# microsoft/YOLaT-VectorGraphicsRecognition

Measured on AMD Instinct MI355X. Metric: graphs_per_sec, higher is better.
Workload: dtype f32

## Files before the change

include/yolat_hip.h:

```cpp
#ifndef YOLAT_HIP_H
#define YOLAT_HIP_H

#include <stddef.h>
#include <stdint.h>

#ifdef __cplusplus
extern "C" {
#endif

typedef void* yolat_stream_t;

#define YOLAT_E_INVALID   (-1)
#define YOLAT_E_UNSUPPORTED (-2)

#define YOLAT_STATUS_EDGE_RANGE  1
#define YOLAT_STATUS_SEG_UNSORTED 2
#define YOLAT_STATUS_SEG_RANGE   4
#define YOLAT_STATUS_NOT_LOCAL   8


int yolat_abi_version(void);
const char* yolat_strerror(int code);


size_t yolat_csr_work_elems(int64_t N, int64_t E);
int yolat_coo_to_csr(const int64_t* edge, int64_t stride_e, int64_t stride_c, int64_t E, int64_t N,
                     int32_t* row_ptr, int32_t* perm, int32_t* src_csr, int32_t* dst_csr,
                     int32_t* work, int32_t* status, yolat_stream_t stream);

size_t yolat_csc_work_elems(int64_t N);
int yolat_csc_by_source(const int32_t* src_csr, int64_t E, int64_t N, int32_t* col_ptr,
                        int32_t* slots, int32_t* work, yolat_stream_t stream);

int yolat_expand_ranges(const int32_t* start, const int32_t* prefix, int64_t S, int64_t total, int32_t* out,
                        yolat_stream_t stream);
size_t yolat_subgraph_work_elems(int64_t N, int64_t n_sub);
int yolat_subgraph_reindex(const int32_t* node_ids, int64_t n_sub, int64_t N, const int64_t* edge,
                           int64_t stride_e, int64_t stride_c, const int32_t* edge_ids, int64_t m_sub,
                           const int64_t* bbox_idx, int64_t* edge_out, int64_t* bbox_idx_out, int32_t* work,
                           int32_t* status, yolat_stream_t stream);
int yolat_gather_rows_bytes(const void* src, int64_t src_row_bytes, const int32_t* idx, int64_t rows,
                            int64_t row_bytes, void* dst, int64_t dst_row_bytes, yolat_stream_t stream);

int yolat_fixup_offsets(int64_t* edge, int64_t E, const int64_t* edge_ptr, int64_t* bbox_idx, int64_t N,
                        const int64_t* node_ptr, const int64_t* node_off, const int64_t* prop_off, int64_t B,
                        yolat_stream_t stream);

int yolat_segment_ptr(const int64_t* bbox_idx, int64_t N, int64_t P, int32_t* seg_ptr,
                      int32_t* node_seg, int32_t* status, yolat_stream_t stream);

size_t yolat_graph_work_elems(int64_t N, int64_t E);
int yolat_graph_prepare(const int64_t* edge, int64_t stride_e, int64_t stride_c, const float* e_attr,
                        const int64_t* bbox_idx, int64_t E, int64_t N, int64_t P, int32_t* row_ptr,
                        int32_t* perm, int32_t* src_csr, int32_t* dst_csr, float* attr_csr,
                        int32_t* seg_ptr, int32_t* node_seg, int32_t* work, int32_t* status,
                        yolat_stream_t stream);

int yolat_graph_prepare_plan(int64_t N, int64_t E, int64_t other_wgs, int32_t* rows, int32_t* csr_wgs);

int yolat_gather_rows(const float* src, int64_t ld_src, const int32_t* idx, int64_t rows,
                      int64_t width, float* dst, int64_t ld_dst, yolat_stream_t stream);


#define YOLAT_STATS_ROWS 32
size_t yolat_bn_stats_elems(int64_t M, int64_t C);
int yolat_linear_fwd(const float* A, int64_t lda, int64_t M, int64_t K,
                     const float* a_scale, const float* a_shift, int a_relu,
                     const float* W, int64_t ldw, const float* bias, int64_t Nout,
                     const float* o_scale, const float* o_shift, int o_relu,
                     float* Y, int64_t ldy, int accumulate, float* stats, yolat_stream_t stream);

int yolat_linear_segmax_fwd(const float* A, int64_t lda, int64_t M, int64_t K, const float* W,
                            int64_t ldw, const float* bias, int64_t Nout, const float* o_scale,
                            const float* o_shift, const int32_t* node_seg, float* pool, int64_t ldpool,
                            yolat_stream_t stream);

int yolat_linear_fwd_wt(const float* A, int64_t lda, int64_t M, int64_t K,
                        const float* Wt, int64_t ldw, int64_t Nout,
                        float* Y, int64_t ldy, int accumulate, yolat_stream_t stream);

size_t yolat_linear_bwd_w_work_elems(int64_t M, int64_t Nout, int64_t K);
int yolat_linear_bwd_w(const float* dY, int64_t lddy, int64_t M, int64_t Nout,
                       const float* A, int64_t lda, int64_t K,
                       const float* a_scale, const float* a_shift, int a_relu,
                       float* dW, int64_t lddw, float* db, int accumulate,
                       float* partial, yolat_stream_t stream);

int yolat_bn_finalize(const float* stats, int64_t M, int64_t C, const float* gamma,
                      const float* beta, float* running_mean, float* running_var,
                      float momentum, float eps, float* save_mean, float* save_invstd,
                      float* scale, float* shift, yolat_stream_t stream);

int yolat_bn_eval_coeffs(const float* gamma, const float* beta, const float* running_mean,
                         const float* running_var, float eps, int64_t C, float* scale,
                         float* shift, yolat_stream_t stream);

int yolat_scale_shift_relu(const float* Y, int64_t ldy, int64_t M, int64_t C, const float* scale,
                           const float* shift, int relu, float* Z, int64_t ldz,
                           yolat_stream_t stream);

size_t yolat_bn_bwd_work_elems(int64_t M, int64_t C);
int yolat_bn_relu_bwd(const float* dZ, int64_t lddz, const float* Y, int64_t ldy, int64_t M,
                      int64_t C, const float* gamma, const float* save_mean,
                      const float* save_invstd, const float* scale, const float* shift, int relu,
                      float* dgamma, float* dbeta, int accumulate, float* dY, int64_t lddy,
                      float* work, yolat_stream_t stream);


int yolat_edge_lin1_fwd(const float* x, int64_t ldx, int64_t N, int64_t Cin,
                        const int32_t* src_csr, const int32_t* dst_csr, const float* attr_csr,
                        int64_t E, const float* W1, int64_t ldw, const float* b1, int64_t C,
                        const float* o_scale, const float* o_shift, int o_relu,
                        float* H1, int64_t ldh, float* stats, yolat_stream_t stream);

int yolat_edge_lin1_bwd_w(const float* dH1, int64_t lddh, int64_t E, int64_t C,
                          const float* x, int64_t ldx, int64_t N, int64_t Cin,
                          const int32_t* src_csr, const int32_t* dst_csr, const float* attr_csr,
                          float* dW1, int64_t lddw, float* db1, int accumulate, float* partial,
                          yolat_stream_t stream);

int yolat_edge_lin1_bwd_x(const float* dH1, int64_t lddh, int64_t E, int64_t C, const float* W1,
                          int64_t ldw, int64_t Cin, float* dG, int64_t lddg,
                          yolat_stream_t stream);

int yolat_edge_scatter_bwd(const float* dG, int64_t lddg, int64_t Cin, const int32_t* row_ptr,
                           const int32_t* col_ptr, const int32_t* slots, int64_t N, float* dX,
                           int64_t lddx, int accumulate, yolat_stream_t stream);

int yolat_edge_mlp2_eval(const float* x, int64_t ldx, int64_t N, int64_t Cin, const int32_t* src_csr,
                         const int32_t* dst_csr, const float* attr_csr, int64_t E, const float* W1,
                         const float* b1, const float* s1, const float* t1, const float* W2,
                         const float* b2, const float* s2, const float* t2, int64_t C, float* H2,
                         int64_t ldh, yolat_stream_t stream);

int yolat_graph_prepare_node_uv(const int64_t* edge, int64_t stride_e, int64_t stride_c, const float* e_attr,
                                const int64_t* bbox_idx, int64_t E, int64_t N, int64_t P, int32_t* row_ptr,
                                int32_t* perm, int32_t* src_csr, int32_t* dst_csr, float* attr_csr,
                                int32_t* seg_ptr, int32_t* node_seg, int32_t* work, int32_t* status, const float* x,
                                int64_t ldx, int64_t Cin, const float* Wuv, const float* uv_bias, const float* Wr,
                                const float* br,
                                const float* Wn, const float* bn, const float* sn, const float* tn, int64_t C,
                                float* UV, int64_t ld_uv, float* f_out, int64_t ld_fo, float* s_out, int64_t ld_so,
                                yolat_stream_t stream);

int yolat_conv_split_w1(const float* W1, int64_t Cin, int64_t C, float* Wuv, float* Wc4, yolat_stream_t stream);
int yolat_node_uv_eval(const float* f_in, int64_t ld_f, const float* s_in, int64_t ld_s, int64_t N, int64_t Cin,
                       const float* Wuv, const float* uv_bias, const float* Wr, const float* br, const float* Wn,
                       const float* bn, const float* sn, const float* tn, int64_t C, float* UV, int64_t ld_uv,
                       float* f_out, int64_t ld_fo, float* s_out, int64_t ld_so, yolat_stream_t stream);
int yolat_edge_uv_lin1_fwd(const float* UV, int64_t ld_uv, const int32_t* src_csr, const int32_t* dst_csr,
                           const float* attr_csr, int64_t E, const float* Wc4, const float* b1, int64_t C,
                           float* H1, int64_t ldh, float* stats, yolat_stream_t stream);

// ... 486 lines not shown
```

yolat_vectorgraphicsrecognition_amd/_lib.py:

```python
import ctypes
import os

_HERE = os.path.dirname(os.path.abspath(__file__))
LIB_PATH = os.environ.get("YOLAT_LIB_PATH") or os.path.join(_HERE, "libyolat_hip.so")

c_p = ctypes.c_void_p
c_i64 = ctypes.c_int64
c_int = ctypes.c_int
c_f = ctypes.c_float
c_sz = ctypes.c_size_t

YOLAT_MAX_LAYERS = 8


class ConvEval(ctypes.Structure):
    _fields_ = ([("Cin", c_i64)] + [(n, c_p) for n in
                                    ("W1", "b1", "s1", "t1", "W2", "b2", "s2", "t2", "Wr", "br", "Wn", "bn", "sn", "tn",
                                     "Wuv", "Wc4", "Wuvf", "uvb", "Wc4f", "t2f")] +
                [("Wfr_x6", c_p * 3), ("tfr", c_p), ("Wn_x6", c_p * 3), ("tn_fold", c_p), ("Wnx", c_p), ("tnx", c_p)])


class ModelEval(ctypes.Structure):
    _fields_ = ([("n_blocks", ctypes.c_int32), ("n_blocks_out", ctypes.c_int32), ("n_classes", ctypes.c_int32),
                 ("reserved", ctypes.c_int32), ("C", c_i64), ("F", c_i64), ("H1", c_i64), ("H2", c_i64),
# ... 60 lines not shown
                ("node", TrainLin), ("bn_node", TrainBn)]


class TrainModel(ctypes.Structure):
    _fields_ = [("n_blocks", ctypes.c_int32), ("n_blocks_out", ctypes.c_int32), ("n_classes", ctypes.c_int32),
                ("half", ctypes.c_int32), ("C", c_i64), ("F", c_i64), ("H1", c_i64), ("H2", c_i64),
                ("conv", TrainConv * YOLAT_MAX_LAYERS), ("fus", TrainLin), ("fus_bn", TrainBn), ("fus_s", TrainLin),
                ("fus_s_bn", TrainBn), ("c1", TrainLin), ("c1_bn", TrainBn), ("c2", TrainLin), ("c2_bn", TrainBn),
                ("c3", TrainLin), ("param_base", c_p), ("grad_base", c_p)]


class AdamArgs(ctypes.Structure):
    _fields_ = [("exp_avg", c_p), ("exp_avg_sq", c_p), ("n", c_i64), ("step", c_i64), ("lr", c_f), ("beta1", c_f),
                ("beta2", c_f), ("eps", c_f), ("weight_decay", c_f), ("grad_scale", c_f)]


class PredictTree(ctypes.Structure):
    _fields_ = [("R", c_i64), ("Ctot", c_i64), ("B", c_i64), ("root_row", c_p), ("root_range", c_p), ("child_ptr", c_p),
                ("child_row", c_p), ("child_range", c_p), ("image_root_ptr", c_p)]


class GraphCsr(ctypes.Structure):
    _fields_ = [("row_ptr", c_p), ("src", c_p), ("dst", c_p), ("attr", c_p), ("seg_ptr", c_p), ("node_seg", c_p)]


SIGNATURES = {
    "yolat_abi_version": (c_int, []),
    "yolat_strerror": (ctypes.c_char_p, [c_int]),
    "yolat_csr_work_elems": (c_sz, [c_i64, c_i64]),
    "yolat_coo_to_csr": (c_int, [c_p, c_i64, c_i64, c_i64, c_i64, c_p, c_p, c_p, c_p, c_p, c_p, c_p]),
    "yolat_edge_mlp2_eval": (c_int, [c_p, c_i64, c_i64, c_i64, c_p, c_p, c_p, c_i64, c_p, c_p, c_p, c_p, c_p, c_p, c_p,
                                      c_p, c_i64, c_p, c_i64, c_p]),
    "yolat_node_side_eval": (c_int, [c_p, c_i64, c_p, c_i64, c_i64, c_i64, c_p, c_p, c_p, c_p, c_p, c_p, c_p, c_i64,
                                      c_p, c_i64, c_i64, c_p, c_i64, c_p, c_i64, c_p]),
    "yolat_fusion_pool_train_saved_elems": (c_sz, [c_i64, c_i64, c_i64]),
    "yolat_fusion_pool_train_work_elems": (c_sz, [c_i64, c_i64, c_i64, c_i64]),
    "yolat_fusion_pool_train_fwd": (c_int, [c_p, c_i64, c_i64, c_i64, c_p, c_p, c_i64, c_p, c_p, c_p, c_p, c_f, c_f,
                                             c_p, c_i64, c_p, c_i64, c_p, c_p, c_p, c_p]),
    "yolat_fusion_pool_train_bwd": (c_int, [c_p, c_i64, c_i64, c_i64, c_p, c_p, c_i64, c_p, c_p, c_p, c_p, c_i64, c_p,
                                             c_i64, c_p, c_p, c_p, c_p, c_p, c_i64, c_p, c_p]),
    "yolat_fusion_pool_train_bwd_parts": (c_int, [c_p, c_i64, c_i64, c_i64, c_p, c_p, c_i64, c_p, c_p, c_p, c_p, c_i64, c_p,
                                                   c_i64, c_p, c_p, c_p, c_p, c_p, c_i64, c_p, c_int, c_p]),
    "yolat_fusion_pool_train_fwd_bf16": (c_int, [c_p, c_i64, c_i64, c_i64, c_p, c_p, c_i64, c_p, c_p, c_p, c_p, c_f, c_f,
                                                  c_p, c_i64, c_p, c_i64, c_p, c_p, c_p, c_p]),
    "yolat_fusion_pool_train_bwd_parts_bf16": (c_int, [c_p, c_i64, c_i64, c_i64, c_p, c_p, c_i64, c_p, c_p, c_p, c_p, c_i64,
                                                        c_p, c_i64, c_p, c_p, c_p, c_p, c_p, c_i64, c_p, c_int, c_p]),
    "yolat_bt_linear_fwd": (c_int, [c_p, c_i64, c_i64, c_i64, c_p, c_p, c_int, c_p, c_i64, c_p, c_i64, c_p, c_i64, c_p, c_p]),
    "yolat_bt_linear_fwd_wt": (c_int, [c_p, c_i64, c_i64, c_i64, c_p, c_i64, c_i64, c_p, c_i64, c_int, c_p]),
    "yolat_bt_linear_bwd_w_work_elems": (c_sz, [c_i64, c_i64, c_i64]),
    "yolat_bt_linear_bwd_w": (c_int, [c_p, c_i64, c_i64, c_i64, c_p, c_i64, c_i64, c_p, c_p, c_int, c_p, c_i64, c_p, c_p,
                                       c_p]),
    "yolat_expand_ranges": (c_int, [c_p, c_p, c_i64, c_i64, c_p, c_p]),
    "yolat_subgraph_work_elems": (c_sz, [c_i64, c_i64]),
    "yolat_subgraph_reindex": (c_int, [c_p, c_i64, c_i64, c_p, c_i64, c_i64, c_p, c_i64, c_p, c_p, c_p, c_p, c_p, c_p]),
    "yolat_gather_rows_bytes": (c_int, [c_p, c_i64, c_p, c_i64, c_i64, c_p, c_i64, c_p]),
    "yolat_fixup_offsets": (c_int, [c_p, c_i64, c_p, c_p, c_i64, c_p, c_p, c_p, c_i64, c_p]),
    "yolat_conv_split_w1": (c_int, [c_p, c_i64, c_i64, c_p, c_p, c_p]),
    "yolat_node_uv_eval": (c_int, [c_p, c_i64, c_p, c_i64, c_i64, c_i64, c_p, c_p, c_p, c_p, c_p, c_p, c_p, c_p, c_i64,
                                    c_p, c_i64, c_p, c_i64, c_p, c_i64, c_p]),
    "yolat_edge_uv_mlp2_eval": (c_int, [c_p, c_i64, c_p, c_p, c_p, c_i64, c_p, c_p, c_p, c_p, c_p, c_p, c_p, c_p, c_i64,
                                         c_p, c_i64, c_p]),
    "yolat_edge_uv_mlp2_mean_eval": (c_int, [c_p, c_i64, c_p, c_p, c_p, c_p, c_i64, c_i64, c_p, c_p, c_p, c_p, c_p, c_p,
                                              c_p, c_p, c_i64, c_p, c_i64, c_p]),
    "yolat_edge_uv_mlp2_mean_eval_variant": (c_int, [c_p, c_i64, c_p, c_p, c_p, c_p, c_i64, c_i64, c_p, c_p, c_p, c_p,
                                                      c_p, c_p, c_p, c_p, c_i64, c_p, c_i64, c_int, c_p]),
    "yolat_edge_uv_sums": (c_int, [c_p, c_i64, c_p, c_p, c_p, c_i64, c_i64, c_p, c_i64, c_p]),
    "yolat_conv_merge_dw1": (c_int, [c_p, c_p, c_i64, c_i64, c_p, c_i64, c_int, c_p]),
    "yolat_fusion_pair_eval": (c_int, [c_p, c_i64, c_i64, c_i64, c_p, c_p, c_p, c_p, c_i64, c_p, c_p, c_i64, c_p, c_i64,
                                        c_i64, c_p, c_p, c_p, c_p, c_p, c_i64, c_p]),
    "yolat_graph_prepare_node_uv": (c_int, [c_p, c_i64, c_i64, c_p, c_p, c_i64, c_i64, c_i64] + [c_p] * 9 +
                                    [c_p, c_i64, c_i64] + [c_p] * 8 + [c_i64, c_p, c_i64, c_p, c_i64, c_p, c_i64, c_p]),
    "yolat_csc_work_elems": (c_sz, [c_i64]),
    "yolat_csc_by_source": (c_int, [c_p, c_i64, c_i64, c_p, c_p, c_p, c_p]),
    "yolat_segment_ptr": (c_int, [c_p, c_i64, c_i64, c_p, c_p, c_p, c_p]),
    "yolat_graph_work_elems": (c_sz, [c_i64, c_i64]),
    "yolat_graph_prepare": (c_int, [c_p, c_i64, c_i64, c_p, c_p, c_i64, c_i64, c_i64, c_p, c_p, c_p, c_p, c_p,
                                    c_p, c_p, c_p, c_p, c_p]),
    "yolat_graph_prepare_plan": (c_int, [c_i64, c_i64, c_i64, c_p, c_p]),
    "yolat_gather_rows": (c_int, [c_p, c_i64, c_p, c_i64, c_i64, c_p, c_i64, c_p]),
    "yolat_bn_stats_elems": (c_sz, [c_i64, c_i64]),
    "yolat_linear_fwd": (c_int, [c_p, c_i64, c_i64, c_i64, c_p, c_p, c_int,
                                 c_p, c_i64, c_p, c_i64, c_p, c_p, c_int,
                                 c_p, c_i64, c_int, c_p, c_p]),
    "yolat_linear_segmax_fwd": (c_int, [c_p, c_i64, c_i64, c_i64, c_p, c_i64, c_p, c_i64, c_p, c_p, c_p, c_p, c_i64,
                                        c_p]),
    "yolat_linear_fwd_wt": (c_int, [c_p, c_i64, c_i64, c_i64, c_p, c_i64, c_i64, c_p, c_i64, c_int, c_p]),
    "yolat_linear_bwd_w_work_elems": (c_sz, [c_i64, c_i64, c_i64]),
    "yolat_linear_bwd_w": (c_int, [c_p, c_i64, c_i64, c_i64, c_p, c_i64, c_i64, c_p, c_p, c_int,
                                   c_p, c_i64, c_p, c_int, c_p, c_p]),
    "yolat_bn_finalize": (c_int, [c_p, c_i64, c_i64, c_p, c_p, c_p, c_p, c_f, c_f, c_p, c_p, c_p, c_p, c_p]),
    "yolat_bn_eval_coeffs": (c_int, [c_p, c_p, c_p, c_p, c_f, c_i64, c_p, c_p, c_p]),
    "yolat_scale_shift_relu": (c_int, [c_p, c_i64, c_i64, c_i64, c_p, c_p, c_int, c_p, c_i64, c_p]),
    "yolat_bn_bwd_work_elems": (c_sz, [c_i64, c_i64]),
    "yolat_bn_relu_bwd": (c_int, [c_p, c_i64, c_p, c_i64, c_i64, c_i64, c_p, c_p, c_p, c_p, c_p, c_int,
                                  c_p, c_p, c_int, c_p, c_i64, c_p, c_p]),
    "yolat_edge_lin1_fwd": (c_int, [c_p, c_i64, c_i64, c_i64, c_p, c_p, c_p, c_i64, c_p, c_i64, c_p,
                                    c_i64, c_p, c_p, c_int, c_p, c_i64, c_p, c_p]),
    "yolat_edge_lin1_bwd_w": (c_int, [c_p, c_i64, c_i64, c_i64, c_p, c_i64, c_i64, c_i64, c_p, c_p, c_p,
                                      c_p, c_i64, c_p, c_int, c_p, c_p]),
    "yolat_edge_lin1_bwd_x": (c_int, [c_p, c_i64, c_i64, c_i64, c_p, c_i64, c_i64, c_p, c_i64, c_p]),
    "yolat_edge_scatter_bwd": (c_int, [c_p, c_i64, c_i64, c_p, c_p, c_p, c_i64, c_p, c_i64, c_int, c_p]),
    "yolat_csr_mean_fwd": (c_int, [c_p, c_i64, c_i64, c_p, c_p, c_int, c_p, c_i64, c_p, c_i64, c_int, c_p]),
    "yolat_csr_mean_bwd": (c_int, [c_p, c_i64, c_i64, c_p, c_p, c_i64, c_p, c_i64, c_p]),
    "yolat_segment_mean_fwd": (c_int, [c_p, c_i64, c_i64, c_p, c_p, c_int, c_p, c_i64, c_p, c_i64, c_p]),
    "yolat_segment_max_fwd": (c_int, [c_p, c_i64, c_i64, c_p, c_p, c_int, c_p, c_i64, c_i64, c_p, c_i64,
                                      c_p, c_p]),
    "yolat_pool_prepare": (c_int, [c_p, c_p, c_i64, c_i64, c_i64, c_p, c_i64, c_p, c_i64, c_p]),
    "yolat_segment_mean_bwd": (c_int, [c_p, c_i64, c_i64, c_p, c_p, c_i64, c_p, c_i64, c_p]),
    "yolat_segment_max_bwd": (c_int, [c_p, c_i64, c_i64, c_p, c_p, c_i64, c_p, c_i64, c_p]),
    "yolat_softmax_ce_work_elems": (c_sz, [c_i64]),
    "yolat_softmax_ce": (c_int, [c_p, c_i64, c_p, c_i64, c_i64, c_p, c_p, c_i64, c_p, c_p]),
    "yolat_sigmoid": (c_int, [c_p, c_i64, c_i64, c_i64, c_p, c_i64, c_p]),
    "yolat_sigmoid_bwd": (c_int, [c_p, c_i64, c_p, c_i64, c_i64, c_i64, c_p, c_i64, c_p]),
    "yolat_bce_work_elems": (c_sz, [c_i64]),
    "yolat_bce": (c_int, [c_p, c_i64, c_p, c_i64, c_i64, c_p, c_p, c_i64, c_p, c_p]),
    "yolat_sigmoid_bce": (c_int, [c_p, c_i64, c_p, c_i64, c_i64, c_p, c_p, c_i64, c_p, c_i64, c_p, c_p]),
    "yolat_adam_step": (c_int, [c_p, c_p, c_p, c_p, c_i64, c_f, c_f, c_f, c_f, c_f, c_i64, c_f, c_p]),
    "yolat_profile_enabled": (c_int, []),
    "yolat_profile_enable": (c_int, [c_int]),
    "yolat_profile_reset": (c_int, []),
    "yolat_profile_count": (c_int, []),
    "yolat_profile_get": (c_int, [c_int, ctypes.c_char_p, c_int, ctypes.POINTER(c_f), ctypes.POINTER(c_int),
                                  ctypes.POINTER(ctypes.c_double), ctypes.POINTER(ctypes.c_double)]),
    "yolat_forward_eval_workspace_bytes": (c_sz, [ctypes.POINTER(ModelEval), c_i64, c_i64, c_i64]),
    "yolat_forward_eval": (c_int, [ctypes.POINTER(ModelEval), c_p, c_i64, c_p, c_i64, c_i64, c_p, c_p, c_i64, c_i64,
                                   c_i64, c_p, c_i64, c_p, c_sz, c_p, c_p]),
    "yolat_forward_eval_primed": (c_int, [ctypes.POINTER(ModelEval), c_p, c_i64, c_p, c_i64, c_i64, c_p, c_p, c_i64,
                                          c_i64, c_i64, c_p, c_i64, c_p, c_sz, c_p, c_p]),
    "yolat_edge_uv_lin1_fwd": (c_int, [c_p, c_i64, c_p, c_p, c_p, c_i64, c_p, c_p, c_i64, c_p, c_i64, c_p, c_p]),
    "yolat_nms_work_bytes": (c_sz, [c_i64]),
    "yolat_nms": (c_int, [c_p, c_p, c_i64, c_f, c_p, c_p, c_p, c_sz, c_p]),
    "yolat_detect_scores": (c_int, [c_p, c_i64, c_i64, c_i64, c_p, c_p, c_i64, c_p, c_int, c_p, c_p]),
    "yolat_nms_batched_work_bytes": (c_sz, [c_i64, c_i64, c_i64]),
    "yolat_nms_batched": (c_int, [c_p, c_i64, c_i64, c_p, c_i64, c_f, c_f, c_int, c_p, c_p, c_p, c_sz, c_p]),
    "yolat_detect_match": (c_int, [c_p, c_p, c_i64, c_p, c_p, c_i64, c_p, c_p, c_i64, c_p, c_p]),
    "yolat_f32_to_bf16": (c_int, [c_p, c_i64, c_p, c_p]),
    "yolat_edge_uv_lin1_fwd_h": (c_int, [c_p, c_i64, c_p, c_p, c_p, c_i64, c_p, c_p, c_i64, c_p, c_i64, c_p, c_p]),
    "yolat_linear_fwd_h": (c_int, [c_p, c_i64, c_i64, c_i64, c_p, c_p, c_int, c_p, c_i64, c_p, c_i64, c_p, c_i64, c_p,
                                   c_p, c_p]),
    "yolat_csr_mean_fwd_h": (c_int, [c_p, c_i64, c_i64, c_p, c_p, c_int, c_p, c_i64, c_p, c_i64, c_int, c_p]),
    "yolat_csr_mean_bwd_h": (c_int, [c_p, c_i64, c_i64, c_p, c_p, c_i64, c_p, c_i64, c_p]),
    "yolat_bn_relu_bwd_h": (c_int, [c_p, c_i64, c_p, c_i64, c_i64, c_i64, c_p, c_p, c_p, c_p, c_int, c_p, c_p, c_int,
                                    c_p, c_i64, c_p, c_p]),
    "yolat_linear_bwd_w_h": (c_int, [c_p, c_i64, c_i64, c_i64, c_p, c_int, c_i64, c_i64, c_p, c_p, c_int, c_p, c_i64,
                                     c_p, c_int, c_p, c_p]),
    "yolat_linear_fwd_wt_h": (c_int, [c_p, c_i64, c_i64, c_i64, c_p, c_i64, c_i64, c_p, c_i64, c_p, c_p]),
    "yolat_edge_uv_sums_h": (c_int, [c_p, c_i64, c_p, c_p, c_p, c_i64, c_i64, c_p, c_i64, c_p]),
    "yolat_split_bf16x3": (c_int, [c_p, c_i64, c_i64, c_i64, c_p, c_p, c_p, c_p, c_p]),
    "yolat_linear_fwd_rows_x6": (c_int, [c_p, c_i64, c_i64, c_i64, c_p, c_p, c_int, c_p, c_i64, c_p, c_i64, c_p, c_i64, c_p,
                                         c_p, c_p]),
    "yolat_node_uv_eval_x6": (c_int, [c_p, c_i64, c_p, c_i64, c_i64, c_p, c_p, c_p, c_p, c_p, c_p, c_p, c_p, c_p, c_i64,
                                      c_p, c_i64, c_p, c_i64, c_p]),
    "yolat_fusion_pair_eval_x6": (c_int, [c_p, c_i64, c_i64, c_i64, c_p, c_p, c_p, c_p, c_i64, c_p, c_p, c_i64, c_p,
                                          c_i64, c_i64, c_p, c_p, c_p, c_p, c_p, c_i64, c_p]),
    "yolat_inv_degree": (c_int, [c_p, c_i64, c_p, c_p]),
    "yolat_bn_csr_work_elems": (c_sz, [c_i64, c_i64]),
    "yolat_bn_csr_bwd_stats": (c_int, [ctypes.POINTER(BnCsrGrad), c_i64, c_i64, c_p, c_p, c_int, c_p, c_p, c_p]),
    "yolat_linear_bwd_w_csr": (c_int, [ctypes.POINTER(BnCsrGrad), c_i64, c_i64, c_p, c_i64, c_i64, c_p, c_p, c_int, c_p,
                                       c_i64, c_p, c_int, c_p, c_p]),
    "yolat_linear_fwd_wt_csr": (c_int, [ctypes.POINTER(BnCsrGrad), c_i64, c_i64, c_p, c_i64, c_i64, c_p, c_i64, c_p]),
    "yolat_bn_csr_l2_bwd_work_elems": (c_sz, []),
    "yolat_bn_csr_l2_bwd": (c_int, [ctypes.POINTER(BnCsrGrad), c_i64, c_p, c_i64, c_p, c_p, c_int, c_p, c_i64, c_p, c_i64,
                                    c_p, c_int, c_p, c_i64, c_p, c_p, c_p, c_p, c_p, c_p, c_p]),
    "yolat_bn_relu_bwd_apply": (c_int, [c_p, c_i64, c_p, c_i64, c_i64, c_i64, c_p, c_p, c_p, c_p, c_int, c_p, c_p, c_i64,
                                        c_int, c_p]),
    "yolat_gemm_x6_packed_elems": (c_sz, [c_i64, c_i64]),
# ... 101 lines not shown
```

yolat_vectorgraphicsrecognition_amd/csrc/forward_eval.hip:

```cpp
#include "common.hpp"

namespace {
struct Plan {
  int* row_ptr; int* perm; int* src; int* dst; float* attr; int* work; int* seg_ptr; int* node_seg;
  float* H1; float* H2; float* UV; float* UV2; float* f_tmp[YOLAT_MAX_LAYERS]; float* s_tmp[YOLAT_MAX_LAYERS];
  float* feats; float* fsup; float* Z; float* c1; float* c2;
  float* gx_work;
  uint16_t* Zs;
  size_t bytes;
};

Plan carve(const yolat_model_eval* m, long N, long E, long P, void* ws) {
  Carver c{reinterpret_cast<char*>(ws), 0};
  Plan p;
  const long C = m->C, F = m->F, D = C * m->n_blocks_out, Ee = E > 0 ? E : 1;
  p.row_ptr = c.take<int>(N + 1); p.perm = c.take<int>(Ee); p.src = c.take<int>(Ee); p.dst = c.take<int>(Ee);
  p.attr = c.take<float>(Ee * 4); p.work = c.take<int>(yolat_graph_work_elems(N, E));
  p.seg_ptr = c.take<int>(P + 1); p.node_seg = c.take<int>(N);
  p.H1 = c.take<float>(Ee * C); p.H2 = c.take<float>(Ee * C); p.UV = c.take<float>(N * 2 * C);
  p.UV2 = (m->n_blocks >= 2 && yl_edge_tile_groups(N, E) == 1) ? c.take<float>(N * 2 * C) : nullptr;
  const int lo = m->n_blocks - m->n_blocks_out;
  for (int l = 0; l < m->n_blocks; ++l) {
    p.f_tmp[l] = (l < lo) ? c.take<float>(N * C) : nullptr;
    p.s_tmp[l] = (l < lo) ? c.take<float>(N * C) : nullptr;
// ... 236 lines not shown
            const yolat_conv_eval& cn = m->conv[l + 1];
            nx.s_in = s_out; nx.ld_si = ld_out;
            nx.Wn = cn.Wn; nx.bn = cn.bn; nx.sn = cn.sn; nx.tn = cn.tn;
            nx.s_out = sn >= 0 ? p.fsup + sn * C : p.s_tmp[l + 1]; nx.ld_so = sn >= 0 ? D : C;
            nx.s_tiles = yl_cdiv(N, 64);
          }
          const bool with_next = nx.Wp != nullptr;
          if (with_next)
            snprintf(nm, sizeof nm, "edge_uv_mlp2_mean+node_uv_next[E x (U+V+attr) -> %ld -> %ld -> mean; N x %ld -> %ld+%ld+%ld]",
                     C, C, C, 2 * C, C, C);
          else
            snprintf(nm, sizeof nm, "edge_uv_mlp2_mean[E x (U+V+attr) -> %ld -> %ld -> mean]", C, C);
          YL_STAGE(nm, 2.0 * E * (4.0 * C + C * C) + (with_next ? 8.0 * N * C * C : 0.0),
                   E * ((2.0 * cv.Cin + 4.0) * 4.0 + 8.0) + 4.0 * N * C + (with_next ? 4.0 * (N * C + 4.0 * N * C) : 0.0),
                   fold ? yl_edge_uv_mlp2_mean_eval_impl(uv_l, 2 * C, p.src, p.dst, p.attr, p.row_ptr, N, E, cv.Wc4f,
                                                         nullptr, nullptr, nullptr, cv.W2, nullptr, cv.s2, cv.t2f, C,
                                                         f_out, ld_out, YOLAT_EDGE_AUTO, rd, &rode,
                                                         nx.Wp ? &nx : nullptr, &did_next, stream)
                        : yl_edge_uv_mlp2_mean_eval_impl(uv_l, 2 * C, p.src, p.dst, p.attr, p.row_ptr, N, E, cv.Wc4,
                                                         cv.b1, cv.s1, cv.t1, cv.W2, cv.b2, cv.s2, cv.t2, C, f_out,
                                                         ld_out, YOLAT_EDGE_AUTO, rd, &rode, nullptr, nullptr, stream));
          if (rode) pool_done |= ride_a.parts;
          next_done = did_next != 0;
          uv_next = nx.UV;
        }
      } else {
      if (E > 0) {
        snprintf(nm, sizeof nm, "edge_mlp2[E x %ld -> %ld -> %ld, gathered]", (long)K1, C, C);
        YL_STAGE(nm, 2.0 * E * (K1 * C + C * C), E * (K1 * 4.0 + 8.0) + 4.0 * E * C,
                 yolat_edge_mlp2_eval(f_in, ld_f, N, cv.Cin, p.src, p.dst, p.attr, E, cv.W1, cv.b1, cv.s1, cv.t1,
                                      cv.W2, cv.b2, cv.s2, cv.t2, C, p.H2, C, stream));
      }
      snprintf(nm, sizeof nm, "node_pair[lin_r | mlp_node, N x %ld -> %ld]", (long)cv.Cin, C);
      YL_STAGE(nm, 4.0 * N * cv.Cin * C, 8.0 * (N * cv.Cin + N * C),
               yolat_node_side_eval(f_in, ld_f, s_in, ld_s, N, cv.Cin, cv.Wr, cv.br, cv.Wn, cv.bn, cv.sn, cv.tn,
                                    nullptr, C, p.row_ptr, 0, C, f_out, ld_out, s_out, ld_out, stream));
      if (E > 0) {
        YL_STAGE("csr_mean[E x C -> N x C]", 1.0 * E * C, 4.0 * (E * C + 2.0 * N * C) + 4.0 * N,
                 yolat_csr_mean_fwd(p.H2, C, C, nullptr, nullptr, 0, p.row_ptr, N, f_out, ld_out, 1, stream));
      }
      }
    } else {
    snprintf(nm, sizeof nm, "lin_r[N x %ld -> %ld]", (long)cv.Cin, C);
    YL_STAGE(nm, 2.0 * N * cv.Cin * C, 4.0 * (N * cv.Cin + N * C + C * cv.Cin),
             yolat_linear_fwd(f_in, ld_f, N, cv.Cin, nullptr, nullptr, 0, cv.Wr, cv.Cin, cv.br, C, nullptr,
                              nullptr, 0, f_out, ld_out, 0, nullptr, stream));
    if (E > 0) {
      snprintf(nm, sizeof nm, "edge_lin1[E x %ld -> %ld, gathered]", (long)K1, C);
      YL_STAGE(nm, 2.0 * E * K1 * C, E * (K1 * 4.0 + 8.0) + 4.0 * E * C,
               yolat_edge_lin1_fwd(f_in, ld_f, N, cv.Cin, p.src, p.dst, p.attr, E, cv.W1, 2 * cv.Cin + 4,
                                   cv.b1, C, cv.s1, cv.t1, 1, p.H1, C, nullptr, stream));
      snprintf(nm, sizeof nm, "edge_lin2[E x %ld -> %ld]", C, C);
      YL_STAGE(nm, 2.0 * E * C * C, 8.0 * E * C,
               yolat_linear_fwd(p.H1, C, E, C, nullptr, nullptr, 0, cv.W2, C, cv.b2, C, cv.s2, cv.t2, 1, p.H2,
                                C, 0, nullptr, stream));
      YL_STAGE("csr_mean[E x C -> N x C]", 1.0 * E * C, 4.0 * (E * C + 2.0 * N * C) + 4.0 * N,
               yolat_csr_mean_fwd(p.H2, C, C, nullptr, nullptr, 0, p.row_ptr, N, f_out, ld_out, 1, stream));
    }
    snprintf(nm, sizeof nm, "mlp_node[N x %ld -> %ld]", (long)cv.Cin, C);
    YL_STAGE(nm, 2.0 * N * cv.Cin * C, 4.0 * (N * cv.Cin + N * C + C * cv.Cin),
             yolat_linear_fwd(s_in, ld_s, N, cv.Cin, nullptr, nullptr, 0, cv.Wn, cv.Cin, cv.bn, C, cv.sn, cv.tn, 1,
                              s_out, ld_out, 0, nullptr, stream));
    }
    f_in = f_out; ld_f = ld_out; s_in = s_out; ld_s = ld_out;
  }

  float* sup = p.Z + 2 * F + D;
  const bool ride_max = ride_b.blocks > 0 && (pool_done & YL_POOL_ZERO);
  const int pool_left = (YL_POOL_ZERO | YL_POOL_MAX | YL_POOL_MEAN) & ~pool_done & ~(ride_max ? YL_POOL_MAX : 0);
  if (pool_left) {
    YL_STAGE("pool_prepare[max(feats), mean(fsup), zero]", 2.0 * N * D, 8.0 * N * D + 4.0 * P * (F + 2 * D),
             yl_pool_prepare_parts(p.feats, p.fsup, D, D, F, p.seg_ptr, P, p.Z, ZW, pool_left, stream));
  }
  snprintf(nm, sizeof nm, "fusion_gemm+segmax[N x %ld -> %ld -> P] | super[P x %ld -> %ld]", D, F, D, F);
  YL_STAGE(nm, 2.0 * (N + P) * D * F, 4.0 * (N * D + 2.0 * D * F + 2.0 * P * F + N + P * D),
           fusion_x6 ? yl_fusion_pair_eval_x6_impl(p.feats, D, N, D, m->Wf_hi, m->Wf_mid, m->Wf_lo, m->tf_fold, F,
                                                   p.node_seg, p.Z, ZW, sup, ZW, P, m->Wfs_hi, m->Wfs_mid, m->Wfs_lo,
                                                   m->tfs_fold, p.Z + F + D, ZW, ride_max ? &ride_b : nullptr, stream)
                     : yolat_fusion_pair_eval(p.feats, D, N, D, m->Wf, m->bf, m->sf, m->tf, F, p.node_seg, p.Z, ZW, sup,
                                              ZW, P, m->Wfs, m->bfs, m->sfs, m->tfs, p.Z + F + D, ZW, stream));
  bool cls_x6 = p.Zs != nullptr && m->H1 % 16 == 0 && m->H2 % 16 == 0;
  for (int i = 0; i < 3; ++i) cls_x6 = cls_x6 && m->Wc_x6[i] != nullptr && m->tc_fold[i] != nullptr;
  const bool cls1_gx = m->Wc1_gx && m->tc1_gx && ZW % 16 == 0 && P >= YOLAT_CLS1_X6_MIN_ROWS;
  snprintf(nm, sizeof nm, "cls1[P x %ld -> %ld]", ZW, (long)m->H1);
  YL_STAGE(nm, 2.0 * P * ZW * m->H1, 4.0 * (P * ZW + ZW * m->H1 + P * m->H1),
           cls1_gx ? yolat_gemm_x6(p.Z, ZW, P, ZW, m->Wc1_gx, m->tc1_gx, 1, m->H1, p.c1, m->H1, p.gx_work, stream)
           : cls_x6 ? cls1_x6(p.Z, ZW, P, p.Zs, m->Wc_x6[0], m->tc_fold[0], m->H1, p.c1, stream)
                  : yolat_linear_fwd(p.Z, ZW, P, ZW, nullptr, nullptr, 0, m->Wc1, ZW, m->bc1, m->H1, m->sc1, m->tc1, 1,
                                     p.c1, m->H1, 0, nullptr, stream));
  snprintf(nm, sizeof nm, "cls2[P x %ld -> %ld]", (long)m->H1, (long)m->H2);
  YL_STAGE(nm, 2.0 * P * m->H1 * m->H2, 4.0 * (P * m->H1 + m->H1 * m->H2 + P * m->H2),
           cls_x6 ? yolat_linear_x6(p.c1, m->H1, P, m->H1, m->Wc_x6[1], m->tc_fold[1], 1, m->H2, p.c2, m->H2, stream)
                  : yolat_linear_fwd(p.c1, m->H1, P, m->H1, nullptr, nullptr, 0, m->Wc2, m->H1, m->bc2, m->H2, m->sc2,
                                     m->tc2, 1, p.c2, m->H2, 0, nullptr, stream));
  snprintf(nm, sizeof nm, "cls3[P x %ld -> %d]", (long)m->H2, (int)m->n_classes);
  YL_STAGE(nm, 2.0 * P * m->H2 * m->n_classes, 4.0 * (P * m->H2 + m->H2 * m->n_classes + P * m->n_classes),
           cls_x6 ? yolat_linear_x6(p.c2, m->H2, P, m->H2, m->Wc_x6[2], m->tc_fold[2], 0, m->n_classes, logits,
                                    ld_logits, stream)
                  : yolat_linear_fwd(p.c2, m->H2, P, m->H2, nullptr, nullptr, 0, m->Wc3, m->H2, m->bc3, m->n_classes,
                                     nullptr, nullptr, 0, logits, ld_logits, 0, nullptr, stream));
  return 0;
}
```

yolat_vectorgraphicsrecognition_amd/ops.py:

```python
import ctypes
import os

import torch

from ._lib import lib, check

STATS_ROWS = 32
STATUS_EDGE_RANGE, STATUS_SEG_UNSORTED, STATUS_SEG_RANGE, STATUS_NOT_LOCAL = 1, 2, 4, 8

_WEIGHT_EPOCH = [0]


def weight_epoch():
    return _WEIGHT_EPOCH[0]


def bump_weight_epoch():
    _WEIGHT_EPOCH[0] += 1


_RAW_STREAM = getattr(torch._C, "_cuda_getCurrentRawStream", None)
_GET_DEVICE = getattr(torch._C, "_cuda_getDevice", None)
_STREAM_OBJ = {}

# ... 212 lines not shown
                                  work.data_ptr(), g.status.data_ptr(), _stream()), "yolat_graph_prepare")
    g._work = work
    return g


def segment_ptr(bbox_idx, num_proposals):
    P, N = int(num_proposals), int(bbox_idx.shape[0])
    dev = bbox_idx.device
    z = torch.zeros(4 + (P + 1 + 3) // 4 * 4 + max(N, 1), dtype=torch.int32, device=dev)
    seg = z[4:4 + P + 1]
    check(lib.yolat_segment_ptr(_i(bbox_idx, torch.int64, "bbox_idx"), N, P, seg.data_ptr(),
                                z[4 + (P + 1 + 3) // 4 * 4:].data_ptr(), z[0:1].data_ptr(), _stream()), "yolat_segment_ptr")
    return seg


def augment_batch(pos, x, seg_ptr, prop_ptr, bbox, params, cols=(3, 4)):
    pos_ptr = _f(pos, "pos")
    N, P, B = int(pos.shape[0]), int(bbox.shape[0]), int(params.shape[0])
    if pos.dim() != 2 or pos.shape[1] != 2 or bbox.dim() != 2 or bbox.shape[1] != 4 or x.dim() != 2 or x.shape[0] != N:
        raise ValueError("augment_batch: pos must be [N,2], x [N,C], bbox [P,4]")
    if (N > 0 and not pos.is_contiguous()) or (P > 0 and not bbox.is_contiguous()):
        raise ValueError("augment_batch: pos and bbox must be contiguous")
    if not params.is_cuda or params.dtype != torch.float64 or params.dim() != 2 or params.shape[1] != 8 or \
            not params.is_contiguous():
        raise TypeError("augment_batch: params must be a contiguous [B,8] float64 CUDA tensor")
    if seg_ptr.shape[0] != P + 1 or prop_ptr.shape[0] != B + 1:
        raise ValueError("augment_batch: seg_ptr must be [P+1] and prop_ptr [B+1]")
    cx, cy = int(cols[0]), int(cols[1])
    if not (0 <= cx < x.shape[1] and 0 <= cy < x.shape[1]) or cx == cy:
        raise ValueError("augment_batch: position columns %r outside x [N,%d]" % (cols, x.shape[1]))
    for t in (x, seg_ptr, prop_ptr, bbox, params):
        if t.device != pos.device:
            raise RuntimeError("augment_batch: every operand must live on %s" % pos.device)
    check(lib.yolat_augment_batch(pos_ptr, _f(x, "x"), _ld(x), cx, cy, _i(seg_ptr, torch.int32, "seg_ptr"),
                                  _i(prop_ptr, torch.int64, "prop_ptr"), _f(bbox, "bbox"), params.data_ptr(), N, P, B,
                                  _stream()), "yolat_augment_batch")



def stats_buffer(M, C, device):
    return torch.empty(int(lib.yolat_bn_stats_elems(M, C)), dtype=torch.float32, device=device)


STRICT_FP32 = os.environ.get("YOLAT_STRICT_FP32", "0") == "1"
X6_TRAIN_GEMM = not STRICT_FP32
X6_TRAIN_ROWS = False


def linear_fwd(A, W, bias, Y, a_pro=None, a_relu=False, o_pro=None, o_relu=False,
               accumulate=False, stats=None):
    M, K = A.shape
    Nout = W.shape[0]
    asc, ash = (a_pro if a_pro is not None else (None, None))
    osc, osh = (o_pro if o_pro is not None else (None, None))
    if _is_h(A) or _is_h(Y):
        if not (_is_h(A) and _is_h(Y)) or o_pro is not None or o_relu or accumulate:
            raise ValueError("bf16-storage linear_fwd: A and Y bfloat16, no output epilogue / accumulation")
        wwork = torch.empty(Nout * K, dtype=torch.bfloat16, device=A.device)
        check(lib.yolat_linear_fwd_h(_h(A, "A"), _ld(A), M, K, _f(asc, "a_scale", True), _f(ash, "a_shift", True),
                                     int(a_relu), _f(W, "W"), _ld(W), _f(bias, "bias", True), Nout, _h(Y, "Y"), _ld(Y),
                                     _f(stats, "stats", True), wwork.data_ptr(), _stream()), "yolat_linear_fwd_h")
        return Y
    if (X6_TRAIN_GEMM and stats is not None and a_pro is None and o_pro is None and not o_relu and not accumulate
            and bias is not None and M >= 1024 and K >= 256 and K % 16 == 0 and Nout >= 128 and _ld(A) % 4 == 0
            and A.data_ptr() % 16 == 0 and int(lib.yolat_gemm_x6_work_elems(M, Nout, K)) == 0):
        packed = torch.empty(int(lib.yolat_gemm_x6_packed_elems(Nout, K)), dtype=torch.bfloat16, device=A.device)
        check(lib.yolat_gemm_x6_pack(_f(W, "W"), _ld(W), Nout, K, None, packed.data_ptr(), _stream()), "yolat_gemm_x6_pack")
        check(lib.yolat_gemm_x6_stats(_f(A, "A"), _ld(A), M, K, packed.data_ptr(), _f(bias, "bias"), Nout, _f(Y, "Y"), _ld(Y),
                                      _f(stats, "stats"), _stream()), "yolat_gemm_x6_stats")
        return Y
    if (X6_TRAIN_ROWS and o_pro is None and not o_relu and not accumulate and bias is not None and M >= 65536
            and K in (64, 128) and Nout % 64 == 0 and _ld(A) % 4 == 0 and A.data_ptr() % 16 == 0):
        wsplit = torch.empty(3 * Nout * K, dtype=torch.bfloat16, device=A.device)
        check(lib.yolat_linear_fwd_rows_x6(_f(A, "A"), _ld(A), M, K, _f(asc, "a_scale", True), _f(ash, "a_shift", True),
                                           int(a_relu), _f(W, "W"), _ld(W), _f(bias, "bias"), Nout, _f(Y, "Y"), _ld(Y),
                                           _f(stats, "stats", True), wsplit.data_ptr(), _stream()),
              "yolat_linear_fwd_rows_x6")
        return Y
    check(lib.yolat_linear_fwd(_f(A, "A"), _ld(A), M, K, _f(asc, "a_scale", True), _f(ash, "a_shift", True),
                               int(a_relu), _f(W, "W"), _ld(W), _f(bias, "bias", True), Nout,
                               _f(osc, "o_scale", True), _f(osh, "o_shift", True), int(o_relu),
                               _f(Y, "Y"), _ld(Y), int(accumulate), _f(stats, "stats", True),
                               _stream()), "yolat_linear_fwd")
    return Y


def linear_fwd_wt(A, Wt, Y, accumulate=False):
    M, K = A.shape
    Nout = Wt.shape[1]
    if _is_h(A) or _is_h(Y):
        if not (_is_h(A) and _is_h(Y)) or accumulate:
            raise ValueError("bf16-storage linear_fwd_wt: A and Y bfloat16, no accumulation")
        wwork = torch.empty(Nout * K, dtype=torch.bfloat16, device=A.device)
        check(lib.yolat_linear_fwd_wt_h(_h(A, "A"), _ld(A), M, K, _f(Wt, "Wt"), _ld(Wt), Nout, _h(Y, "Y"), _ld(Y),
                                        wwork.data_ptr(), _stream()), "yolat_linear_fwd_wt_h")
        return Y
    if (X6_TRAIN_GEMM and not accumulate and M >= 1024 and K >= 256 and K % 16 == 0 and Nout >= 512
            and _ld(A) % 4 == 0 and A.data_ptr() % 16 == 0):
        packed = torch.empty(int(lib.yolat_gemm_x6_packed_elems(Nout, K)), dtype=torch.bfloat16, device=A.device)
        check(lib.yolat_gemm_x6_pack_t(_f(Wt, "Wt"), _ld(Wt), Nout, K, packed.data_ptr(), _stream()),
              "yolat_gemm_x6_pack_t")
        work = torch.empty(max(1, int(lib.yolat_gemm_x6_work_elems(M, Nout, K))), dtype=torch.float32, device=A.device)
        check(lib.yolat_gemm_x6(_f(A, "A"), _ld(A), M, K, packed.data_ptr(), None, 0, Nout, _f(Y, "Y"), _ld(Y),
                                work.data_ptr(), _stream()), "yolat_gemm_x6")
        return Y
    check(lib.yolat_linear_fwd_wt(_f(A, "A"), _ld(A), M, K, _f(Wt, "Wt"), _ld(Wt), Nout, _f(Y, "Y"),
                                  _ld(Y), int(accumulate), _stream()), "yolat_linear_fwd_wt")
    return Y



def _bt_aligned(t):
    return t if t.data_ptr() % 16 == 0 else t.clone()


def _bt_check(rc, what, shape):
    if rc == -2:
        raise ValueError("bf16_dense training: %s does not take %s" % (what, shape))
    check(rc, what)


def bt_linear_fwd(A, W, bias, Y, a_pro=None, a_relu=False, stats=None):
    M, K = A.shape
    Nout = W.shape[0]
    asc, ash = (a_pro if a_pro is not None else (None, None))
    W = _bt_aligned(W)
    _bt_check(lib.yolat_bt_linear_fwd(_f(A, "A"), _ld(A), M, K, _f(asc, "a_scale", True), _f(ash, "a_shift", True),
                                      int(a_relu), _f(W, "W"), _ld(W), _f(bias, "bias", True), Nout, _f(Y, "Y"), _ld(Y),
                                      _f(stats, "stats", True), _stream()), "yolat_bt_linear_fwd",
              "[%d, %d] x [%d, %d]^T" % (M, K, Nout, K))
    return Y


def bt_linear_fwd_wt(A, Wt, Y, accumulate=False):
    M, K = A.shape
    Nout = Wt.shape[1]
    Wt = _bt_aligned(Wt)
    _bt_check(lib.yolat_bt_linear_fwd_wt(_f(A, "A"), _ld(A), M, K, _f(Wt, "Wt"), _ld(Wt), Nout, _f(Y, "Y"), _ld(Y),
                                         int(accumulate), _stream()), "yolat_bt_linear_fwd_wt",
              "[%d, %d] x [%d, %d]" % (M, K, K, Nout))
    return Y


def bt_linear_bwd_w(dY, A, dW, db=None, a_pro=None, a_relu=False):
    M, Nout = dY.shape
    K = A.shape[1]
    asc, ash = (a_pro if a_pro is not None else (None, None))
    work = torch.empty(int(lib.yolat_bt_linear_bwd_w_work_elems(M, Nout, K)), dtype=torch.float32, device=dY.device)
    _bt_check(lib.yolat_bt_linear_bwd_w(_f(dY, "dY"), _ld(dY), M, Nout, _f(A, "A"), _ld(A), K, _f(asc, "a_scale", True),
                                        _f(ash, "a_shift", True), int(a_relu), _f(dW, "dW"), _ld(dW), _f(db, "db", True),
                                        work.data_ptr(), _stream()), "yolat_bt_linear_bwd_w",
              "[%d, %d]^T x [%d, %d]" % (M, Nout, M, K))
    return dW


def linear_bwd_w(dY, A, dW, db=None, a_pro=None, a_relu=False, accumulate=False):
    M, Nout = dY.shape
    K = A.shape[1]
    asc, ash = (a_pro if a_pro is not None else (None, None))
    work = torch.empty(int(lib.yolat_linear_bwd_w_work_elems(M, Nout, K)), dtype=torch.float32,
                       device=dY.device)
    if _is_h(dY):
        check(lib.yolat_linear_bwd_w_h(_h(dY, "dY"), _ld(dY), M, Nout, _h(A, "A") if _is_h(A) else _f(A, "A"),
                                       int(_is_h(A)), _ld(A), K, _f(asc, "a_scale", True), _f(ash, "a_shift", True),
                                       int(a_relu), _f(dW, "dW"), _ld(dW), _f(db, "db", True), int(accumulate),
                                       work.data_ptr(), _stream()), "yolat_linear_bwd_w_h")
# ... 625 lines not shown
```

Before: 16080.

## Add split-K bf16x6 MFMA GEMM for small-grid cls1 classifier layer

Adds a new kernel for the cls1 linear layer, used when the output tile grid is small (under 160 tiles of 64x64) and K is large. Each 32x32 tile is computed by 8 waves that split K across the block, with async global-to-LDS double buffering. The fp32 products are emulated with six bf16 MFMAs from a three-way split, and the partial sums are reduced in LDS before a fused bias/scale/relu epilogue. The aim is more parallelism and matrix-core throughput than the generic fp32 path on a skinny GEMM, at the cost of extra MFMA work, an LDS reduction and a small numeric difference from strict fp32.

```diff
diff --git a/include/yolat_hip.h b/include/yolat_hip.h
--- a/include/yolat_hip.h
+++ b/include/yolat_hip.h
@@ -69,6 +69,10 @@
                      const float* W, int64_t ldw, const float* bias, int64_t Nout,
                      const float* o_scale, const float* o_shift, int o_relu,
                      float* Y, int64_t ldy, int accumulate, float* stats, yolat_stream_t stream);
+
+int yolat_linear_sk_x6(const float* A, int64_t lda, int64_t M, int64_t K, const float* W, int64_t ldw, const float* bias,
+                       int64_t Nout, const float* o_scale, const float* o_shift, int o_relu, float* Y, int64_t ldy,
+                       yolat_stream_t stream);
 
 int yolat_linear_segmax_fwd(const float* A, int64_t lda, int64_t M, int64_t K, const float* W,
                             int64_t ldw, const float* bias, int64_t Nout, const float* o_scale,
diff --git a/yolat_vectorgraphicsrecognition_amd/_lib.py b/yolat_vectorgraphicsrecognition_amd/_lib.py
--- a/yolat_vectorgraphicsrecognition_amd/_lib.py
+++ b/yolat_vectorgraphicsrecognition_amd/_lib.py
@@ -166,6 +166,7 @@
     "yolat_linear_fwd": (c_int, [c_p, c_i64, c_i64, c_i64, c_p, c_p, c_int,
                                  c_p, c_i64, c_p, c_i64, c_p, c_p, c_int,
                                  c_p, c_i64, c_int, c_p, c_p]),
+    "yolat_linear_sk_x6": (c_int, [c_p, c_i64, c_i64, c_i64, c_p, c_i64, c_p, c_i64, c_p, c_p, c_int, c_p, c_i64, c_p]),
     "yolat_linear_segmax_fwd": (c_int, [c_p, c_i64, c_i64, c_i64, c_p, c_i64, c_p, c_i64, c_p, c_p, c_p, c_p, c_i64,
                                         c_p]),
     "yolat_linear_fwd_wt": (c_int, [c_p, c_i64, c_i64, c_i64, c_p, c_i64, c_i64, c_p, c_i64, c_int, c_p]),
diff --git a/yolat_vectorgraphicsrecognition_amd/csrc/forward_eval.hip b/yolat_vectorgraphicsrecognition_amd/csrc/forward_eval.hip
--- a/yolat_vectorgraphicsrecognition_amd/csrc/forward_eval.hip
+++ b/yolat_vectorgraphicsrecognition_amd/csrc/forward_eval.hip
@@ -342,10 +342,14 @@
   bool cls_x6 = p.Zs != nullptr && m->H1 % 16 == 0 && m->H2 % 16 == 0;
   for (int i = 0; i < 3; ++i) cls_x6 = cls_x6 && m->Wc_x6[i] != nullptr && m->tc_fold[i] != nullptr;
   const bool cls1_gx = m->Wc1_gx && m->tc1_gx && ZW % 16 == 0 && P >= YOLAT_CLS1_X6_MIN_ROWS;
+  static const bool sk_x6_on = []() { const char* v = getenv("YOLAT_CLS1_SK_X6"); return !(v && v[0] == '0'); }();
+  const bool cls1_sk = sk_x6_on && !cls1_gx && !cls_x6 && !yl_strict_fp32() && ZW >= 1024 && ZW % 128 == 0 &&
+                       (long)yl_cdiv(P, 64) * yl_cdiv(m->H1, 64) < 160 && yl_aligned16(p.Z) && yl_aligned16(m->Wc1);
   snprintf(nm, sizeof nm, "cls1[P x %ld -> %ld]", ZW, (long)m->H1);
   YL_STAGE(nm, 2.0 * P * ZW * m->H1, 4.0 * (P * ZW + ZW * m->H1 + P * m->H1),
            cls1_gx ? yolat_gemm_x6(p.Z, ZW, P, ZW, m->Wc1_gx, m->tc1_gx, 1, m->H1, p.c1, m->H1, p.gx_work, stream)
            : cls_x6 ? cls1_x6(p.Z, ZW, P, p.Zs, m->Wc_x6[0], m->tc_fold[0], m->H1, p.c1, stream)
+           : cls1_sk ? yolat_linear_sk_x6(p.Z, ZW, P, ZW, m->Wc1, ZW, m->bc1, m->H1, m->sc1, m->tc1, 1, p.c1, m->H1, stream)
                   : yolat_linear_fwd(p.Z, ZW, P, ZW, nullptr, nullptr, 0, m->Wc1, ZW, m->bc1, m->H1, m->sc1, m->tc1, 1,
                                      p.c1, m->H1, 0, nullptr, stream));
   snprintf(nm, sizeof nm, "cls2[P x %ld -> %ld]", (long)m->H1, (long)m->H2);
diff --git a/yolat_vectorgraphicsrecognition_amd/csrc/linear_sk_x6.hip b/yolat_vectorgraphicsrecognition_amd/csrc/linear_sk_x6.hip
--- /dev/null
+++ b/yolat_vectorgraphicsrecognition_amd/csrc/linear_sk_x6.hip
@@ -0,0 +1,112 @@
+#include "x6.hpp"
+
+__global__ void __launch_bounds__(512) k_gemm_nt_sk_x6dma(const float* __restrict__ A, long lda, int rowsA,
+                                                         const float* __restrict__ B, long ldb, int rowsB, Epilogue ep,
+                                                         int M, int N, int K, long long* stamps) {
+  constexpr int NW = 8, BT = 32, BK = 128, NP = 32 / NW;
+  __shared__ __attribute__((aligned(16))) float smem[2][2][BT * BK];
+  const int tid = threadIdx.x, lane = tid & 63;
+  const int wave = __builtin_amdgcn_readfirstlane(tid >> 6);
+  const int l31 = lane & 31, lhi = lane >> 5;
+  int rt_, ct_;
+  yl_xcd_tile(rt_, ct_);
+  const int row0 = rt_ * BT, col0 = ct_ * BT;
+  const EpiPre pre = epi_prefetch(ep, row0, col0 + l31, M, N);
+  f32x16 acc;
+#pragma unroll
+  for (int r = 0; r < 16; ++r) acc[r] = 0.f;
+  const unsigned lds0 = (unsigned)(size_t)&smem[0][0][0];
+  const float* src[NP];
+#pragma unroll
+  for (int j = 0; j < NP; ++j) {
+    const int i = NP * wave + j, op = i >> 4, pair = i & 15;
+    const int r = 2 * pair + (lane >> 5), g = (lane & 31) ^ (r & 15);
+    src[j] = op == 0 ? A + (long)yl_min(row0 + r, rowsA - 1) * lda + 4 * g : B + (long)yl_min(col0 + r, rowsB - 1) * ldb + 4 * g;
+  }
+  auto stage = [&](int s, int k0) {
+#pragma unroll
+    for (int j = 0; j < NP; ++j) {
+      const int i = NP * wave + j, op = i >> 4, pair = i & 15;
+      yl_glds16(src[j] + k0, lds0 + (unsigned)(((s * 2 + op) * BT * BK + pair * 256) * 4));
+    }
+  };
+  const int g0 = 4 * wave + 2 * lhi;
+  const int off0 = l31 * BK + 4 * (g0 ^ (l31 & 15)), off1 = l31 * BK + 4 * ((g0 + 1) ^ (l31 & 15));
+  auto compute = [&](int s) {
+    const float* As = &smem[s][0][0];
+    const float* Bs = &smem[s][1][0];
+    const float4 a0 = *reinterpret_cast<const float4*>(As + off0), a1 = *reinterpret_cast<const float4*>(As + off1);
+    const float4 b0 = *reinterpret_cast<const float4*>(Bs + off0), b1 = *reinterpret_cast<const float4*>(Bs + off1);
+    const float a8[8] = {a0.x, a0.y, a0.z, a0.w, a1.x, a1.y, a1.z, a1.w};
+    const float b8[8] = {b0.x, b0.y, b0.z, b0.w, b1.x, b1.y, b1.z, b1.w};
+    fx_bf16x8 ah, am, al, bh, bm, bl;
+    fx_split8(a8, ah, am, al);
+    fx_split8(b8, bh, bm, bl);
+    acc = __builtin_amdgcn_mfma_f32_32x32x16_bf16(ah, bl, acc, 0, 0, 0);
+    acc = __builtin_amdgcn_mfma_f32_32x32x16_bf16(al, bh, acc, 0, 0, 0);
+    acc = __builtin_amdgcn_mfma_f32_32x32x16_bf16(am, bm, acc, 0, 0, 0);
+    acc = __builtin_amdgcn_mfma_f32_32x32x16_bf16(am, bh, acc, 0, 0, 0);
+    acc = __builtin_amdgcn_mfma_f32_32x32x16_bf16(ah, bm, acc, 0, 0, 0);
+    acc = __builtin_amdgcn_mfma_f32_32x32x16_bf16(ah, bh, acc, 0, 0, 0);
+  };
+  const int nch = K / BK;
+  long long t0 = 0, t_wait = 0, t_comp = 0;
+  const bool st_on = stamps != nullptr && tid == 0;
+  stage(0, 0);
+  for (int kc = 0; kc < nch; ++kc) {
+    long long ta = 0, tb = 0, tc = 0;
+    if (kc + 1 < nch) {
+      stage((kc + 1) & 1, (kc + 1) * BK);
+      if (st_on) ta = clock64();
+      asm volatile("s_waitcnt vmcnt(4)" ::: "memory");
+    } else {
+      if (st_on) ta = clock64();
+      asm volatile("s_waitcnt vmcnt(0)" ::: "memory");
+    }
+    asm volatile("s_waitcnt lgkmcnt(0)\n\ts_barrier" ::: "memory");
+    if (st_on) tb = clock64();
+    compute(kc & 1);
+    asm volatile("s_waitcnt lgkmcnt(0)\n\ts_barrier" ::: "memory");
+    if (st_on) { tc = clock64(); t_wait += tb - ta; t_comp += tc - tb; if (kc == 0) t0 = ta; }
+  }
+  if (st_on) {
+    const long o = 3 * (blockIdx.x + (long)gridDim.x * blockIdx.y);
+    stamps[o] = t_wait; stamps[o + 1] = t_comp; stamps[o + 2] = clock64() - t0;
+  }
+  float* red = &smem[0][0][0];
+  if (wave > 0) {
+#pragma unroll
+    for (int r = 0; r < 16; ++r) red[((wave - 1) * 16 + r) * 64 + lane] = acc[r];
+  }
+  __syncthreads();
+  if (wave == 0) {
+#pragma unroll
+    for (int w = 0; w < NW - 1; ++w)
+#pragma unroll
+      for (int r = 0; r < 16; ++r) acc[r] += red[(w * 16 + r) * 64 + lane];
+    wave_epilogue(acc, row0, col0 + l31, lhi, ep, M, N, pre);
+  }
+}
+
+static bool yl_linear_sk_x6_ok(const float* A, int64_t lda, int64_t M, int64_t K, const float* W, int64_t ldw, int64_t Nout) {
+  return M > 0 && Nout > 0 && K >= 128 && K % 128 == 0 && K < (1LL << 31) && lda % 4 == 0 && ldw % 4 == 0 && yl_aligned16(A) &&
+         yl_aligned16(W) && M <= 65536 && Nout <= 65536;
+}
+
+extern "C" int yolat_linear_sk_x6(const float* A, int64_t lda, int64_t M, int64_t K, const float* W, int64_t ldw,
+                                  const float* bias, int64_t Nout, const float* o_scale, const float* o_shift, int o_relu,
+                                  float* Y, int64_t ldy, yolat_stream_t stream) {
+  if (M < 0 || K <= 0 || Nout <= 0 || (M > 0 && (!A || !Y)) || !W) return YOLAT_E_INVALID;
+  if (M >= (1LL << 31) || lda < K || ldw < K || ldy < Nout) return YOLAT_E_INVALID;
+  if ((o_scale == nullptr) != (o_shift == nullptr)) return YOLAT_E_INVALID;
+  if (M == 0) return 0;
+  if (!yl_linear_sk_x6_ok(A, lda, M, K, W, ldw, Nout)) return YOLAT_E_UNSUPPORTED;
+  Epilogue ep;
+  ep.bias = bias; ep.scale = o_scale; ep.shift = o_shift; ep.relu = o_relu;
+  ep.Y = Y; ep.ldy = ldy; ep.accumulate = 0; ep.stats = nullptr; ep.seg = nullptr; ep.pool = nullptr; ep.ldpool = 0;
+  const dim3 grid(yl_cdiv(M, 32), yl_cdiv(Nout, 32));
+  hipLaunchKernelGGL(k_gemm_nt_sk_x6dma, grid, dim3(512), 0, (hipStream_t)stream, A, (long)lda, (int)M, W, (long)ldw, (int)Nout,
+                     ep, (int)M, (int)Nout, (int)K, yl_gemm_sk_dma_stamps());
+  YL_LAUNCH_CHECK();
+  return 0;
+}
diff --git a/yolat_vectorgraphicsrecognition_amd/ops.py b/yolat_vectorgraphicsrecognition_amd/ops.py
--- a/yolat_vectorgraphicsrecognition_amd/ops.py
+++ b/yolat_vectorgraphicsrecognition_amd/ops.py
@@ -318,6 +318,16 @@
                                _f(osc, "o_scale", True), _f(osh, "o_shift", True), int(o_relu),
                                _f(Y, "Y"), _ld(Y), int(accumulate), _f(stats, "stats", True),
                                _stream()), "yolat_linear_fwd")
+    return Y
+
+
+def linear_sk_x6(A, W, bias, Y, o_pro=None, o_relu=False):
+    M, K = A.shape
+    Nout = W.shape[0]
+    osc, osh = (o_pro if o_pro is not None else (None, None))
+    check(lib.yolat_linear_sk_x6(_f(A, "A"), _ld(A), M, K, _f(W, "W"), _ld(W), _f(bias, "bias", True), Nout,
+                                 _f(osc, "o_scale", True), _f(osh, "o_shift", True), int(o_relu), _f(Y, "Y"), _ld(Y),
+                                 _stream()), "yolat_linear_sk_x6")
     return Y
 
 
```

Result: faster. 16620 (median of 6 runs) (+3.3%).
